# PlasmaControl/spectrogram-enhancement

Hardware: AMD Instinct MI355X
Metric: spectrograms/s (STFT+VAE-denoise fwd) at 1/2/4/8 GPUs; PSNR vs CPU ref (higher is better)
Workload: dtype fp16; 1 GPU; BASELINE config 5 per GPU: end-to-end STFT -> SVD -> autoencoder-denoise inference stream, 16,512-sample fp16 shots -> specgr 128x128 (256 hann / hop 128) -> denoiseSignal default -> 3-layer conv AE (16/32/64, 5x5) fp16 forward -> fp16 reconstructions (32,768 B per shot); shots_per_launch=2048, samples=16512, stft_dtype=fp32, svd_dtype=fp32 (fp64 small algebra), ae_dtype=fp16, parallelism=shot-sharded x1, streams_per_gpu=2

## Files before the change

### spectrogram-enhancement_amd/csrc/conv_rows.hip

```cpp
#include <hip/hip_runtime.h>

#include <algorithm>
#include <cstdint>
#include <mutex>
#include <string>
#include <type_traits>

#include "lds_dma.hpp"
#include "specenh.h"
#include "runtime.hpp"

namespace specenh {
int set_error(int code, const std::string& msg);

namespace {

typedef _Float16 f16x8 __attribute__((ext_vector_type(8)));
typedef __bf16 bf16x8 __attribute__((ext_vector_type(8)));
typedef float f32x4 __attribute__((ext_vector_type(4)));

template <typename T>
__device__ __forceinline__ f32x4 mfma(const uint4& a, const uint4& b, f32x4 acc) {
  if constexpr (__is_same(T, _Float16))
    return __builtin_amdgcn_mfma_f32_16x16x32_f16(__builtin_bit_cast(f16x8, a),
// ... 947 lines not shown
      f32x4 acc[4] = {bias, bias, bias, bias};
#pragma unroll
      for (int dy = DY0; dy <= DY1; ++dy) {
        const unsigned char* src = ring + ((g + dy - DY0) & 7) * C::ROWB;
#pragma unroll
        for (int dx = DY0; dx <= DY1; ++dx) {
          if (!C::any_tap(dy, dx)) continue;
          const uint4 b = *reinterpret_cast<const uint4*>(src + xo[dx - DY0]);
#pragma unroll
          for (int ph = 0; ph < 4; ++ph)
            if (C::tap(ph, dy, dx)) acc[ph] = mfma<T>(wf[C::tap_index(ph, dy, dx)], b, acc[ph]);
        }
      }
#pragma unroll
      for (int ph = 0; ph < 4; ++ph) pk[ph] = relu_pack4<T>(acc[ph]);
      const long long n = (long long)blockIdx.x + (long long)il * G;
      po = ((n * 2 * H + 2 * s) * OW + 2 * (16 * wx + m)) * CO + 16 * nb + 4 * kg;
      held = true;
    }
    if (mk[0] >= 0) wait_vmcnt_ss<15>(vmn - mk[0]);
    lds_barrier();
#pragma unroll
    for (int i = 0; i < LEAD; ++i) mk[i] = mk[i + 1];
    if (++s == SPI) { s = 0; ++il; }
    if (++sp == SPI) { sp = 0; ++ilp; }
  }
  store_held();
}

template <typename T, int CO, int W, int K>
hipError_t launch_convt_rows32(const CRArgs& a, hipStream_t st) {
  using C = TC32<CO, W, K>;
  constexpr int LEAD = 8 - C::NDY - 1 < 3 ? 8 - C::NDY - 1 : 3;
  const void* k = reinterpret_cast<const void*>(&convt_rows32_kernel<T, CO, W, K, LEAD>);
  static int per_cu[64] = {};
  int dev = 0;
  hipError_t e = hipGetDevice(&dev);
  if (e != hipSuccess) return e;
  if (dev < 0 || dev >= 64) dev = 0;
  if (per_cu[dev] == 0) {
    int pc = 0;
    e = hipOccupancyMaxActiveBlocksPerMultiprocessor(&pc, k, C::THREADS, C::LDS);
    if (e != hipSuccess) return e;
    per_cu[dev] = std::max(1, pc);
  }
  const long long grid = std::min<long long>(a.N, (long long)per_cu[dev] * device_cus());
  SPECENH_LAUNCH((convt_rows32_kernel<T, CO, W, K, LEAD>), dim3((unsigned)grid),
                 dim3(C::THREADS), C::LDS, st, a);
  return hipGetLastError();
}

constexpr int C1W = 128;
constexpr int C1CW = 72;
constexpr int C1ROW = 2 * C1CW;
constexpr int C1RING = 16;
constexpr int C1LDS = C1RING * C1ROW * 4;

template <typename T>
__global__ __launch_bounds__(256) void conv1_rows_pool_kernel(CRArgs a) {
  extern __shared__ __attribute__((aligned(16))) unsigned char ring_raw[];
  uint32_t* const ring = reinterpret_cast<uint32_t*>(ring_raw);
  const int tid = threadIdx.x, lane = tid & 63;
  const int wv = __builtin_amdgcn_readfirstlane(tid >> 6);
  const int m = lane & 15, kg = lane >> 4;
  const int H = a.H, SPI = H / 2 + 2, PPI = H + 4;
  const int G = gridDim.x;
  const int nimg = ((int)a.N - (int)blockIdx.x + G - 1) / G;
  const int S = nimg * SPI;

  for (int e = tid; e < C1RING * C1ROW; e += 256) ring[e] = 0u;
  uint4 w0, w1;
  {
    const T* __restrict__ Wg = reinterpret_cast<const T*>(a.w);
    uint32_t q0[4], q1[4];
#pragma unroll
    for (int i = 0; i < 4; ++i) {
      float v[4];
#pragma unroll
      for (int h = 0; h < 2; ++h) {
        const int kx = 2 * i + h;
        v[2 * h] = kx < 5 ? (float)Wg[(m * 5 + kg) * 5 + kx] : 0.f;
        v[2 * h + 1] = kx < 5 && kg == 0 ? (float)Wg[(m * 5 + 4) * 5 + kx] : 0.f;
      }
      q0[i] = pack2<T>(v[0], v[2]);
      q1[i] = pack2<T>(v[1], v[3]);
    }
    w0 = uint4{q0[0], q0[1], q0[2], q0[3]};
    w1 = uint4{q1[0], q1[1], q1[2], q1[3]};
  }
  const f32x4 bias = f32x4{a.b[4 * kg], a.b[4 * kg + 1], a.b[4 * kg + 2], a.b[4 * kg + 3]};

  const T* __restrict__ X = reinterpret_cast<const T*>(a.x);
  auto stage = [&](int pp) -> int {
    if (wv != 0) return 0;
    int nd = 0;
#pragma unroll
    for (int j = 0; j < 2; ++j) {
      const int pos = pp + j;
      const int il = pos / PPI, r = pos - il * PPI - 2;
      uint32_t* dst = ring + (pos & (C1RING - 1)) * C1ROW + 4;
      if (il < nimg && r >= 0 && r < H) {
        const long long n = (long long)blockIdx.x + (long long)il * G;
        if (lane < 16) lds_dma16(X + (n * H + r) * C1W + 8 * lane, dst);
        ++nd;
      } else if (lane < 16) {
        *reinterpret_cast<uint4*>(dst + 4 * lane) = uint4{0u, 0u, 0u, 0u};
      }
    }
    return nd;
  };
  auto shift = [&](int pp) {
    if (tid < 2 * C1CW) {
      const int j = tid / C1CW, i = tid - j * C1CW;
      uint32_t* row = ring + ((pp + j) & (C1RING - 1)) * C1ROW;
      const uint32_t lo = row[i], hi = row[i + 1];
      row[C1CW + i] = __builtin_amdgcn_alignbit(hi, lo, 16);
    }
  };
  __syncthreads();
  for (int pp = 0; pp < 10; pp += 2) stage(pp);
  asm volatile("s_waitcnt vmcnt(0)" ::: "memory");
  lds_barrier();
  shift(0); shift(2); shift(4);
  lds_barrier();

  const int wbase = 16 * wv + m + 3;
  auto bfrag = [&](int pos, int cb) -> uint4 {
    const uint32_t* row = ring + ((pos + kg) & (C1RING - 1)) * C1ROW + cb * C1CW + wbase;
    return uint4{row[0], row[1], row[2], row[3]};
  };
  T* __restrict__ O = reinterpret_cast<T*>(a.out);
  const int PW = C1W / 2, PH = H / 2;
  for (int g = 0; g < S; ++g) {
    const int nd = stage(2 * g + 10);
    shift(2 * g + 6);
    const int il = g / SPI, p = g - il * SPI;
    if (p < PH) {
      const int pb = 2 * g;
      f32x4 acc[2][2];
#pragma unroll
      for (int dy = 0; dy < 2; ++dy)
#pragma unroll
        for (int cb = 0; cb < 2; ++cb) {
          const uint4 b = bfrag(pb + dy, cb);
          uint4 b4 = bfrag(pb + dy + 4, cb);
          if (kg != 0) b4 = uint4{0u, 0u, 0u, 0u};
          acc[dy][cb] = mfma<T>(w0, b, bias);
          acc[dy][cb] = mfma<T>(w1, b4, acc[dy][cb]);
        }
      float v[4];
#pragma unroll
      for (int i = 0; i < 4; ++i)
        v[i] = fmaxf(fmaxf(fmaxf(acc[0][0][i], acc[0][1][i]), fmaxf(acc[1][0][i], acc[1][1][i])),
                     0.f);
      const long long n = (long long)blockIdx.x + (long long)il * G;
      *reinterpret_cast<uint2*>(O + ((n * PH + p) * PW + 16 * wv + m) * 16 + 4 * kg) =
          uint2{pack2<T>(v[0], v[1]), pack2<T>(v[2], v[3])};
    }
    if (wv == 0) {
      const int younger = nd + (p < PH ? 1 : 0);
      if (younger == 0) asm volatile("s_waitcnt vmcnt(0)" ::: "memory");
      else if (younger == 1) asm volatile("s_waitcnt vmcnt(1)" ::: "memory");
      else if (younger == 2) asm volatile("s_waitcnt vmcnt(2)" ::: "memory");
      else asm volatile("s_waitcnt vmcnt(3)" ::: "memory");
    }
    lds_barrier();
  }
}

template <typename T>
hipError_t launch_conv1_rows(const CRArgs& a, hipStream_t st) {
  const void* k = reinterpret_cast<const void*>(&conv1_rows_pool_kernel<T>);
  static int per_cu[64] = {};
  int dev = 0;
  hipError_t e = hipGetDevice(&dev);
  if (e != hipSuccess) return e;
  if (dev < 0 || dev >= 64) dev = 0;
  if (per_cu[dev] == 0) {
    int pc = 0;
    e = hipOccupancyMaxActiveBlocksPerMultiprocessor(&pc, k, 256, C1LDS);
    if (e != hipSuccess) return e;
    per_cu[dev] = std::max(1, pc);
  }
  const long long grid = std::min<long long>(a.N, (long long)per_cu[dev] * device_cus());
  SPECENH_LAUNCH(conv1_rows_pool_kernel<T>, dim3((unsigned)grid), dim3(256), C1LDS, st, a);
  return hipGetLastError();
}

struct E2Args {
  const void* x;
  const void* w1;
  const float* b1;
  const void* w2;
  const float* b2;
  void* out;
  int N, H;
};

constexpr int E2R1 = 32;
#ifndef SPECENH_ENC2_COPIES
#define SPECENH_ENC2_COPIES 4
#endif
constexpr int E2NC = SPECENH_ENC2_COPIES;
__host__ __device__ constexpr int E2CB(int c) {
  return E2NC == 4 ? (c == 0 ? 0 : c == 1 ? 72 : c == 2 ? 178 : 250) : c * C1CW;
}
constexpr int E2ROW = E2NC == 4 ? 352 : 2 * C1CW;
constexpr int E2RROWS = E2R1 + 2;
#ifndef SPECENH_ENC2_STAGGER
#define SPECENH_ENC2_STAGGER 0
#endif

template <typename T, int WPE>
__global__ __launch_bounds__(512) __attribute__((amdgpu_waves_per_eu(WPE)))
void enc2_rows_kernel(E2Args a) {
  using C = RC<16, 32, 64>;
  extern __shared__ __attribute__((aligned(16))) unsigned char lds[];
  unsigned char* const ring = lds;
  uint32_t* const ring1 = reinterpret_cast<uint32_t*>(lds + C::LDS);
  const int tid = threadIdx.x, lane = tid & 63;
  const int wv = __builtin_amdgcn_readfirstlane(tid >> 6);
  const int m = lane & 15, kg = lane >> 4;
  const int wx = wv % C::NWIN, nb = wv / C::NWIN;
  const int x0 = 16 * wx;
  const int H1 = a.H, H = H1 / 2;
  const int SPI = H / 2 + 1, PPI = H1 + 4;
  const int G = gridDim.x;
  const int nimg = ((int)a.N - (int)blockIdx.x + G - 1) / G;
  const int S = nimg * SPI + 1;

  for (int e = tid; e < (C::LDS + E2RROWS * E2ROW * 4) / 16; e += 512)
    reinterpret_cast<uint4*>(lds)[e] = uint4{0u, 0u, 0u, 0u};
  float* const btab = reinterpret_cast<float*>(lds + C::LDS + E2RROWS * E2ROW * 4);
  if (tid < 16) btab[tid] = a.b1[tid];
  else if (tid < 48) btab[tid] = a.b2[tid - 16];
  auto bias2_ld = [&]() { return *reinterpret_cast<const f32x4*>(btab + 16 + 16 * nb + 4 * kg); };

  uint4 wf[13];
  {
    const T* __restrict__ Wg = reinterpret_cast<const T*>(a.w2);
    const int co = 16 * nb + m, hi = kg >> 1, c8 = 8 * (kg & 1);
    auto tap = [&](int ky, int kx) {
      return *reinterpret_cast<const uint4*>(Wg + ((co * 5 + ky) * 5 + kx) * 16 + c8);
    };
#pragma unroll
    for (int ky = 0; ky < 5; ++ky) {
      wf[ky] = tap(ky, hi);
      wf[5 + ky] = tap(ky, 2 + hi);
    }
    wf[10] = tap(hi, 4);
    wf[11] = tap(2 + hi, 4);
    wf[12] = hi ? uint4{0u, 0u, 0u, 0u} : tap(4, 4);
  }

  const int boff = (x0 + m + (kg >> 1)) * 32 + 16 * (kg & 1);
  const int fo = (x0 + m + 4) * 32 + 16 * (kg & 1);
  const int foff = fo + (kg >> 1) * C::ROWB, foffw = fo - (kg >> 1) * 7 * C::ROWB;

  uint4 v0, v1;
  {
    const T* __restrict__ W1 = reinterpret_cast<const T*>(a.w1);
    uint32_t q0[4], q1[4];
#pragma unroll
    for (int i = 0; i < 4; ++i) {
      float v[4];
#pragma unroll
      for (int h = 0; h < 2; ++h) {
        const int kx = 2 * i + h;
        v[2 * h] = kx < 5 ? (float)W1[(m * 5 + kg) * 5 + kx] : 0.f;
        v[2 * h + 1] = kx < 5 && kg == 0 ? (float)W1[(m * 5 + 4) * 5 + kx] : 0.f;
      }
      q0[i] = pack2<T>(v[0], v[2]);
      q1[i] = pack2<T>(v[1], v[3]);
    }
    v0 = uint4{q0[0], q0[1], q0[2], q0[3]};
    v1 = uint4{q1[0], q1[1], q1[2], q1[3]};
  }
  resident_loads_landed();
  const int w1x = wv & 3, jr = wv >> 2;
  const int wbase = 16 * w1x + m + 3;
  const int p1 = 16 * w1x + m;
  const int c4hi = 2 * ((p1 + 3) & 1), w4 = p1 + 3 - ((p1 + 3) & 1);
  const int cbase0 = E2CB(c4hi) + w4, cbase1 = E2CB(1 + c4hi) + w4;

  const T* __restrict__ X = reinterpret_cast<const T*>(a.x);
  auto stage1_at = [&](int pos, int il, int y) -> int {
    uint32_t* dst = ring1 + (pos & (E2R1 - 1)) * E2ROW + 4;
    if (il < nimg && y >= 0 && y < H1) {
      const long long n = (long long)blockIdx.x + (long long)il * G;
      if (lane < 16) lds_dma16_s(X + (n * H1 + y) * C1W, 16u * lane, dst);
      return 1;
    }
    int z = 0;
    asm volatile("" : "+v"(z));
    if (lane < 16) *reinterpret_cast<uint4*>(dst + 4 * lane) = uint4{(uint32_t)z, (uint32_t)z, (uint32_t)z, (uint32_t)z};
    return 0;
  };
  auto stage1 = [&](int pp) -> int {
    if (wv >= 4) return 0;
    const int pos = pp + wv;
    const int il = pos / PPI;
    return stage1_at(pos, il, pos - il * PPI - 2);
  };
  auto shift1 = [&](int pp) {
    constexpr int NW = E2NC == 4 ? C1CW - 2 : C1CW;
    if (tid < 4 * NW) {
      const int j = tid / NW, i = tid - j * NW;
      uint32_t* row = ring1 + ((pp + j) & (E2R1 - 1)) * E2ROW;
      const uint32_t r0 = row[i], r1 = row[i + 1];
      row[E2CB(1) + i] = __builtin_amdgcn_alignbit(r1, r0, 16);
      if constexpr (E2NC == 4) {
        const uint32_t r2 = row[i + 2];
        row[E2CB(2) + i] = r1;
        row[E2CB(3) + i] = __builtin_amdgcn_alignbit(r2, r1, 16);
      }
    }
  };
  auto run_at = [&](const uint32_t* row, int cb) -> uint4 {
    if constexpr (E2NC == 4) {
      typedef __attribute__((address_space(3))) const volatile unsigned long long lds_u64;
      const lds_u64* r = (const lds_u64*)(row + (cb ? cbase1 : cbase0));
      const unsigned long long lo = r[0], hi = r[1];
      return uint4{(uint32_t)lo, (uint32_t)(lo >> 32), (uint32_t)hi, (uint32_t)(hi >> 32)};
    } else {
      const uint32_t* r = row + cb * C1CW + wbase;
      return uint4{r[0], r[1], r[2], r[3]};
    }
  };
  auto bfrag = [&](int pos, int cb) -> uint4 {
    return run_at(ring1 + ((pos + kg) & (E2R1 - 1)) * E2ROW, cb);
  };
  auto bfrag4 = [&](int pos, int cb) -> uint4 {
    const uint32_t* zrow = ring1 + (E2NC == 4 ? E2R1 + 1 - (pos & 1) : E2R1) * E2ROW;
    return run_at(kg == 0 ? ring1 + (pos & (E2R1 - 1)) * E2ROW : zrow, cb);
  };
  auto produce = [&](int g2, int il, int q2) {
    const int r = 2 * q2 + jr;
    const int pb = 4 * g2 + 2 * jr;
    float v[4] = {0.f, 0.f, 0.f, 0.f};
    const f32x4 bias1 = *reinterpret_cast<const f32x4*>(btab + 4 * kg);
#pragma unroll
    for (int dy = 0; dy < 2; ++dy)
#pragma unroll
      for (int cb = 0; cb < 2; ++cb) {
        const uint4 b = bfrag(pb + dy, cb);
        const uint4 b4 = bfrag4(pb + dy + 4, cb);
        f32x4 acc1 = mfma<T>(v0, b, bias1);
        acc1 = mfma<T>(v1, b4, acc1);
#pragma unroll
        for (int i = 0; i < 4; ++i) v[i] = fmaxf(v[i], acc1[i]);
      }
    const bool real = il < nimg && r < H;
    const uint2 pk = real ? uint2{pack2<T>(v[0], v[1]), pack2<T>(v[2], v[3])} : uint2{0u, 0u};
    *reinterpret_cast<uint2*>(ring + ((2 * g2 + jr) & 7) * C::ROWB + (16 * w1x + m + 2) * 32 +
                              8 * kg) = pk;
  };

  __syncthreads();
  for (int pp = 0; pp < 32; pp += 4) stage1(pp);
  asm volatile("s_waitcnt vmcnt(0)" ::: "memory");
  lds_barrier();
  for (int pp = 0; pp < 16; pp += 4) shift1(pp);
  lds_barrier();
  produce(0, 0, 0);
  produce(1, 1 / SPI, 1 % SPI);
  lds_barrier();

  f32x4 acc[6];
#pragma unroll
  for (int i = 0; i < 6; ++i) acc[i] = bias2_ld();
  T* __restrict__ O = reinterpret_cast<T*>(a.out);
  const int PW = 32, PHh = H / 2;
  int c_1 = 0, c_2 = 0;
  auto fdiv = [](int x, int d) { return x >= 0 ? x / d : -((-x + d - 1) / d); };
  int ilA = fdiv(-2, SPI), qA = -2 - ilA * SPI;
  int qC = 0;
  int ilB = 2 / SPI, qB = 2 - ilB * SPI;
  int ilD = (32 + wv) / PPI, rD = 32 + wv - ilD * PPI;
  auto adv = [](int& il, int& q, int by, int per) {
    q += by;
    if (q >= per) { q -= per; ++il; }
  };

  auto step = [&](auto ic, const int s) {
    constexpr int I = decltype(ic)::value;
    auto slot = [](int d) { return (2 * I + d + 12) % 6; };
    int ns = 0;
    {
      f32x4& r0 = acc[slot(-4)];
      f32x4& r1 = acc[slot(-3)];
      {
        const int il = ilA, q = qA;
        if (il >= 0 && il < nimg && q < PHh) {
          ns = 1;
          float v[4];
#pragma unroll
          for (int i = 0; i < 4; ++i) v[i] = fmaxf(max_pair(fmaxf(r0[i], r1[i])), 0.f);
          const long long n = (long long)blockIdx.x + (long long)il * G;
          const long long o = ((n * PHh + q) * PW + (x0 + m) / 2) * 32 + 16 * nb + 4 * kg;
          *reinterpret_cast<uint2*>(O + o) = uint2{pack2<T>(v[0], v[1]), pack2<T>(v[2], v[3])};
        }
      }
      const f32x4 bias = bias2_ld();
      r0 = bias;
// ... 20 lines not shown
      for (int ky = 0; ky < 5; ++ky) {
        f32x4& ac = acc[slot(j + 2 - ky)];
        ac = mfma<T>(wf[5 + ky], b2, ac);
      }
      acc[slot(j + 2)] = mfma<T>(wf[10], bF, acc[slot(j + 2)]);
      acc[slot(j)] = mfma<T>(wf[11], bF, acc[slot(j)]);
      acc[slot(j - 2)] = mfma<T>(wf[12], bF, acc[slot(j - 2)]);
      if (j == 0) {
        uint4 bT = *reinterpret_cast<const uint4*>(ring + ((2 * s) & 7) * C::ROWB + fo);
        if (kg < 2 || q != 0) bT = uint4{0u, 0u, 0u, 0u};
        acc[slot(1)] = mfma<T>(wf[10], bT, acc[slot(1)]);
      }
    }
    };
    if (SPECENH_ENC2_STAGGER && wv >= 4) {
      conv2_rows();
      produce(s + 2, ilB, qB);
    } else {
      produce(s + 2, ilB, qB);
      conv2_rows();
    }
    if (wv < 4) {
      const int younger = c_2 + c_1 + ns + nd;
      if (younger >= 6) {
        asm volatile("s_waitcnt vmcnt(6)" ::: "memory");
      } else switch (younger) {
        case 0: asm volatile("s_waitcnt vmcnt(0)" ::: "memory"); break;
        case 1: asm volatile("s_waitcnt vmcnt(1)" ::: "memory"); break;
        case 2: asm volatile("s_waitcnt vmcnt(2)" ::: "memory"); break;
        case 3: asm volatile("s_waitcnt vmcnt(3)" ::: "memory"); break;
        case 4: asm volatile("s_waitcnt vmcnt(4)" ::: "memory"); break;
        case 5: asm volatile("s_waitcnt vmcnt(5)" ::: "memory"); break;
        default: asm volatile("s_waitcnt vmcnt(6)" ::: "memory"); break;
      }
    }
    c_2 = c_1;
    c_1 = ns + nd;
    adv(ilA, qA, 1, SPI);
    qC = qC + 1 == SPI ? 0 : qC + 1;
    adv(ilB, qB, 1, SPI);
    adv(ilD, rD, 4, PPI);
    lds_barrier();
  };
  int s = 0;
  for (; s + 3 <= S; s += 3) {
    step(std::integral_constant<int, 0>{}, s);
    step(std::integral_constant<int, 1>{}, s + 1);
    step(std::integral_constant<int, 2>{}, s + 2);
  }
  if (s < S) step(std::integral_constant<int, 0>{}, s);
  if (s + 1 < S) step(std::integral_constant<int, 1>{}, s + 1);
}

constexpr int E2LDS = RC<16, 32, 64>::LDS + E2RROWS * E2ROW * 4 + 48 * 4;

template <typename T, int WPE>
hipError_t launch_enc2_wpe(const E2Args& a, hipStream_t st) {
  const void* k = reinterpret_cast<const void*>(&enc2_rows_kernel<T, WPE>);
  static int per_cu[64] = {};
  int dev = 0;
  hipError_t e = hipGetDevice(&dev);
  if (e != hipSuccess) return e;
  if (dev < 0 || dev >= 64) dev = 0;
  if (per_cu[dev] == 0) {
    int pc = 0;
    e = hipOccupancyMaxActiveBlocksPerMultiprocessor(&pc, k, 512, E2LDS);
    if (e != hipSuccess) return e;
    per_cu[dev] = std::max(1, pc);
  }
  const long long grid = std::min<long long>(a.N, (long long)per_cu[dev] * device_cus());
  SPECENH_LAUNCH((enc2_rows_kernel<T, WPE>), dim3((unsigned)grid), dim3(512), E2LDS, st, a);
  return hipGetLastError();
}

template <typename T>
hipError_t launch_enc2(const E2Args& a, hipStream_t st) {
  return variant(V_ENC2_WPE2) ? launch_enc2_wpe<T, 2>(a, st) : launch_enc2_wpe<T, 4>(a, st);
}

}

int conv_rows_pool(int dtype, const void* x, int N, int H, int W, int CI, const void* w,
                   const float* b, int CO, int K, void* out, hipStream_t st, bool* launched) {
  *launched = false;
  if (variant(V_CONV_NO_ROWS) != 0 || N <= 0 || H < 2 || (H & 1) || !b) return SPECENH_OK;
  if ((long long)N * H * W * CI >= (1ll << 31)) return SPECENH_OK;
  CRArgs a{};
  a.x = x; a.w = w; a.b = b; a.out = out; a.N = N; a.H = H;
  hipError_t e = hipSuccess;
  const bool f16 = dtype == SPECENH_DTYPE_F16;
  if (dtype != SPECENH_DTYPE_F16 && dtype != SPECENH_DTYPE_BF16) return SPECENH_OK;
  if (CI == 16 && CO == 32 && W == 64 && K == 5)
    e = f16 ? launch_rows<_Float16, 16, 32, 64>(a, st) : launch_rows<__bf16, 16, 32, 64>(a, st);
  else if (CI == 32 && CO == 64 && W == 32 && K == 5)
    e = f16 ? launch_rows<_Float16, 32, 64, 32>(a, st) : launch_rows<__bf16, 32, 64, 32>(a, st);
  else if (CI == 32 && CO == 32 && W == 64 && K == 5)
    e = f16 ? launch_rows<_Float16, 32, 32, 64>(a, st) : launch_rows<__bf16, 32, 32, 64>(a, st);
  else if (CI == 32 && CO == 32 && W == 64 && K == 3)
    e = f16 ? launch_rows<_Float16, 32, 32, 64, 3>(a, st) : launch_rows<__bf16, 32, 32, 64, 3>(a, st);
  else
    return SPECENH_OK;
  if (e != hipSuccess) return set_error(SPECENH_EHIP, std::string("conv_rows: ") + hipGetErrorString(e));
  *launched = true;
  return SPECENH_OK;
}

}

namespace specenh {

int convt_rows(int dtype, const void* x, int N, int H, int W, int CI, const void* w,
               const float* b, int CO, int K, void* out, hipStream_t st, bool* launched) {
  *launched = false;
  if (variant(V_CONVT_NO_ROWS) != 0 || N <= 0 || H <= 0 || !b) return SPECENH_OK;
  if (dtype != SPECENH_DTYPE_F16 && dtype != SPECENH_DTYPE_BF16) return SPECENH_OK;
  if ((long long)N * 4 * H * W * CO >= (1ll << 31)) return SPECENH_OK;
  CRArgs a{};
  a.x = x; a.w = w; a.b = b; a.out = out; a.N = N; a.H = H;
  const bool f16 = dtype == SPECENH_DTYPE_F16;
  hipError_t e;
  if (CI == 32) {
    if (CO != 32 || W != 32) return SPECENH_OK;
    if (K == 3) e = f16 ? launch_convt_rows32<_Float16, 32, 32, 3>(a, st) : launch_convt_rows32<__bf16, 32, 32, 3>(a, st);
    else if (K == 5) e = f16 ? launch_convt_rows32<_Float16, 32, 32, 5>(a, st) : launch_convt_rows32<__bf16, 32, 32, 5>(a, st);
    else if (K == 7) e = f16 ? launch_convt_rows32<_Float16, 32, 32, 7>(a, st) : launch_convt_rows32<__bf16, 32, 32, 7>(a, st);
    else return SPECENH_OK;
    if (e != hipSuccess) return set_error(SPECENH_EHIP, std::string("convt_rows32: ") + hipGetErrorString(e));
    *launched = true;
    return SPECENH_OK;
  }
// ... 5 lines not shown
  else if (CO == 64 && W == 16)
    e = f16 ? launch_convt_rows<_Float16, 64, 16>(a, st) : launch_convt_rows<__bf16, 64, 16>(a, st);
  else if (CO == 32 && W == 32)
    e = f16 ? launch_convt_rows<_Float16, 32, 32>(a, st) : launch_convt_rows<__bf16, 32, 32>(a, st);
  else
    return SPECENH_OK;
  if (e != hipSuccess) return set_error(SPECENH_EHIP, std::string("convt_rows: ") + hipGetErrorString(e));
  *launched = true;
  return SPECENH_OK;
}

}

namespace specenh {

int conv1_rows_pool(int dtype, const void* x, int N, int H, int W, const void* w,
                    const float* b, int CO, void* out, hipStream_t st, bool* launched) {
  *launched = false;
  if (variant(V_CONV1_NO_ROWS) != 0 || N <= 0 || H < 2 || (H & 1) || W != C1W || CO != 16 || !b)
    return SPECENH_OK;
  if (dtype != SPECENH_DTYPE_F16 && dtype != SPECENH_DTYPE_BF16) return SPECENH_OK;
  if (((uintptr_t)x & 15) || (long long)N * H * W >= (1ll << 31)) return SPECENH_OK;
  CRArgs a{};
  a.x = x; a.w = w; a.b = b; a.out = out; a.N = N; a.H = H;
  const hipError_t e = dtype == SPECENH_DTYPE_F16 ? launch_conv1_rows<_Float16>(a, st)
                                                  : launch_conv1_rows<__bf16>(a, st);
  if (e != hipSuccess) return set_error(SPECENH_EHIP, std::string("conv1_rows: ") + hipGetErrorString(e));
  *launched = true;
  return SPECENH_OK;
}

}

extern "C" int specenh_encoder2(int dtype, const void* x, int N, int H, int W, const void* w1_gemm,
                                const float* b1, int CO1, const void* w2_gemm, const float* b2,
                                int CO2, int k, void* out, void* stream) {
  using namespace specenh;
  if (N < 0 || H <= 0 || W <= 0) return set_error(SPECENH_EINVAL, "bad input shape");
  if (dtype != SPECENH_DTYPE_F16 && dtype != SPECENH_DTYPE_BF16)
    return set_error(SPECENH_EUNSUPPORTED, "fused encoder: fp16 / bf16 only");
  if (W != C1W || CO1 != 16 || CO2 != 32 || k != 5 || (H & 3))
    return set_error(SPECENH_EUNSUPPORTED,
                     "fused encoder: Conv2D(16, 5) + pool + Conv2D(32, 5) + pool on 128-wide "
                     "one-channel images, height a multiple of 4");
  if (N == 0) return SPECENH_OK;
  if (!x || !w1_gemm || !b1 || !w2_gemm || !b2 || !out) return set_error(SPECENH_EINVAL, "null pointer");
  if (((uintptr_t)x & 15) || (long long)N * H * W >= (1ll << 31))
    return set_error(SPECENH_EINVAL, "input must be 16-byte aligned and below 2^31 elements");
  E2Args a{};
  a.x = x; a.w1 = w1_gemm; a.b1 = b1; a.w2 = w2_gemm; a.b2 = b2; a.out = out; a.N = N; a.H = H;
  hipStream_t st = (hipStream_t)stream;
  static std::once_flag once;
  std::call_once(once, [] {
    const void* const ks[4] = {reinterpret_cast<const void*>(&enc2_rows_kernel<_Float16, 4>),
                               reinterpret_cast<const void*>(&enc2_rows_kernel<__bf16, 4>),
                               reinterpret_cast<const void*>(&enc2_rows_kernel<_Float16, 2>),
                               reinterpret_cast<const void*>(&enc2_rows_kernel<__bf16, 2>)};
    for (const void* k : ks)
      (void)hipFuncSetAttribute(k, hipFuncAttributeMaxDynamicSharedMemorySize, E2LDS);
  });
  const hipError_t e = dtype == SPECENH_DTYPE_F16 ? launch_enc2<_Float16>(a, st)
                                                  : launch_enc2<__bf16>(a, st);
  if (e != hipSuccess) return set_error(SPECENH_EHIP, std::string("encoder2: ") + hipGetErrorString(e));
  return SPECENH_OK;
}
```

### spectrogram-enhancement_amd/csrc/runtime.hip

```cpp
#include "runtime.hpp"

#include <atomic>
#include <cstdlib>
#include <cstring>
#include <mutex>
#include <string>

#include "specenh.h"

namespace specenh {
int set_error(int code, const std::string& msg);

namespace {

struct VariantName {
  const char* name;
  int dflt;
};
constexpr VariantName kVariants[V_COUNT] = {
    {"CONVT_PAIR", 0},      {"PATCH_NO_WL", 0},      {"PATCH_NO_K5", 0},
    {"PATCH_WSPLIT", -1},   {"CONV_NO_S2", 0},       {"CONV_NO_PATCH", 0},
    {"CONV_NO_C1MFMA", 0},  {"CONV_NO_NARROW", 0},   {"WGRAD_GENERIC", 0},
    {"WGRAD_NO_CO1", 0},    {"WGRAD_PERPHASE", 0},   {"SVD_GRAM_TILES", 0},
    {"TAIL_TILES", 0},      {"DECODER_UNFUSED", 0},  {"SVD_NO_TOP1", 0},
    {"CONV_NO_ROWS", 0},    {"CONVT_NO_ROWS", 0},    {"CONV1_NO_ROWS", 0},
    {"ENCODER_UNFUSED", 0},  {"STFT_NO_HOLD", 0},    {"D3_MAP", 0},
    {"ENC2_WPE2", 0},        {"CONVT_SHARED_RING", 0}, {"SVD_RECON_VALU", 0},
    {"ROWS_SHORT_LEAD", 0},  {"SVD_GRAM_F32", 0},
    {"SVD_RECON_BLOCKS", 0}, {"CONVT_PG", 0}, {"SVD_GZ_ROWS", 0}, {"EIG_SPLIT", 0}, {"CO1_VALU", 0},
    {"C1_MASK_MFMA", 1}, {"S2_MIN_NT", 2}, {"PATCH_MIN_WG", 512}, {"WGRAD_WG", 1024}, {"WGRAD_C1_TILES", 4},
    {"EIG_GRID", 32}, {"ROWS_BANDS", -1},
};

std::atomic<int> g_variant[V_COUNT];
std::once_flag g_variant_once;

void init_variants() {
  for (int i = 0; i < V_COUNT; ++i) {
    int v = kVariants[i].dflt;
    std::string env = std::string("SPECENH_") + kVariants[i].name;
    if (const char* s = std::getenv(env.c_str()); s && *s) v = std::atoi(s);
    g_variant[i].store(v, std::memory_order_relaxed);
  }
}

int variant_index(const char* name) {
  if (!name) return -1;
  if (std::strncmp(name, "SPECENH_", 8) == 0) name += 8;
  for (int i = 0; i < V_COUNT; ++i)
    if (std::strcmp(name, kVariants[i].name) == 0) return i;
  return -1;
}

constexpr int kMaxDevices = 64;
std::atomic<int> g_cus[kMaxDevices];

constexpr int kRing = 256;
thread_local const void* g_ring[kRing];
thread_local long long g_launches = 0;

}

int variant(Variant v) {
  std::call_once(g_variant_once, init_variants);
  return g_variant[v].load(std::memory_order_relaxed);
}

int device_cus() {
  int dev = 0;
  if (hipGetDevice(&dev) != hipSuccess || dev < 0 || dev >= kMaxDevices) return 256;
  int c = g_cus[dev].load(std::memory_order_relaxed);
  if (c > 0) return c;
  if (hipDeviceGetAttribute(&c, hipDeviceAttributeMultiprocessorCount, dev) != hipSuccess || c <= 0)
    c = 256;
  g_cus[dev].store(c, std::memory_order_relaxed);
  return c;
}

void note_launch(const void* kernel) { g_ring[g_launches++ % kRing] = kernel; }

}

extern "C" {

// ... 67 lines not shown
```

### spectrogram-enhancement_amd/csrc/runtime.hpp

```cpp
#pragma once

#include <hip/hip_runtime.h>

namespace specenh {

enum Variant : int {
  V_CONVT_PAIR = 0,
  V_PATCH_NO_WL,
  V_PATCH_NO_K5,
  V_PATCH_WSPLIT,
  V_CONV_NO_S2,
  V_CONV_NO_PATCH,
  V_CONV_NO_C1MFMA,
  V_CONV_NO_NARROW,
  V_WGRAD_GENERIC,
  V_WGRAD_NO_CO1,
  V_WGRAD_PERPHASE,
  V_SVD_GRAM_TILES,
  V_TAIL_TILES,
  V_DECODER_UNFUSED,
  V_SVD_NO_TOP1,
  V_CONV_NO_ROWS,
  V_CONVT_NO_ROWS,
  V_CONV1_NO_ROWS,
  V_ENCODER_UNFUSED,
  V_STFT_NO_HOLD,
  V_D3_MAP,
  V_ENC2_WPE2,
  V_CONVT_SHARED_RING,
  V_SVD_RECON_VALU,
  V_ROWS_SHORT_LEAD,
  V_SVD_GRAM_F32,
  V_SVD_RECON_BLOCKS,
  V_CONVT_PG,
  V_SVD_GZ_ROWS,
  V_EIG_SPLIT,
  V_CO1_VALU,
  V_C1_MASK_MFMA,
  V_S2_MIN_NT,
  V_PATCH_MIN_WG,
  V_WGRAD_WG,
  V_WGRAD_C1_TILES,
  V_EIG_GRID,
  V_ROWS_BANDS,
  V_COUNT
};

int variant(Variant v);

int device_cus();

void note_launch(const void* kernel);

}

#define SPECENH_LAUNCH(K, ...)                                        \
  do {                                                                \
    ::specenh::note_launch(reinterpret_cast<const void*>(&K));        \
    hipLaunchKernelGGL(K, __VA_ARGS__);                               \
  } while (0)
```

### spectrogram-enhancement_amd/csrc/svd_denoise.hip

```cpp
#include <hip/hip_runtime.h>

#include <algorithm>
#include <cmath>
#include <cstdlib>
#include <string>
#include <vector>

#include "fft_common.hpp"
#include "specenh.h"
#include "runtime.hpp"

namespace specenh {
int set_error(int code, const std::string& msg);

typedef float f32x16 __attribute__((ext_vector_type(16)));

struct XView {
  const float* base;
  long long batch_stride;
  long long sk, si;
};

__global__ __launch_bounds__(256) void gram_kernel(XView x, int K, int r, float* G,
                                                   int ntiles_side) {
// ... 2764 lines not shown
  if (e != hipSuccess) return e;
  SPECENH_LAUNCH((recon_kernel<KP, TO>), dim3((Kr + RB - 1) / RB, (unsigned)nb), dim3(256),
                     lds, st, xb, Kr, r, V, K, lo, hi, comp, only, reinterpret_cast<TO*>(out),
                     ob, osk, osi);
  return hipGetLastError();
}

template <typename TO>
hipError_t launch_recon_k(int KP, XView xb, int Kr, int r, const float* V, int K, int lo,
                          int hi, int comp, const int* only, void* out, long long ob,
                          long long osk, long long osi, long long nb, hipStream_t st) {
  switch (KP) {
#define SPECENH_RC(n)                                                                          \
  case n:                                                                                      \
    return launch_recon_t<n, TO>(xb, Kr, r, V, K, lo, hi, comp, only, out, ob, osk, osi, nb, \
                                 st);
    SPECENH_RC(8) SPECENH_RC(16) SPECENH_RC(24) SPECENH_RC(32) SPECENH_RC(40) SPECENH_RC(48)
#undef SPECENH_RC
    default: return hipErrorInvalidValue;
  }
}

hipError_t launch_recon(int KP, XView xb, int Kr, int r, const float* V, int K, int lo, int hi,
                        int comp, const int* only, void* out, long long ob, long long osk,
                        long long osi, long long nb, hipStream_t st, int odt = SPECENH_DTYPE_F32) {
  if (odt == SPECENH_DTYPE_F16)
    return launch_recon_k<_Float16>(KP, xb, Kr, r, V, K, lo, hi, comp, only, out, ob, osk, osi, nb, st);
  if (odt == SPECENH_DTYPE_BF16)
    return launch_recon_k<__bf16>(KP, xb, Kr, r, V, K, lo, hi, comp, only, out, ob, osk, osi, nb, st);
  return launch_recon_k<float>(KP, xb, Kr, r, V, K, lo, hi, comp, only, out, ob, osk, osi, nb, st);
}

size_t dtype_size(int dt) { return dt == SPECENH_DTYPE_F32 ? 4 : 2; }

struct EigLayout {
  int r;
  long long ld;
  size_t per_matrix() const {
    return (size_t)r * r * 8 + 3 * (size_t)r * 8 + 4 * (size_t)r * ld * 8 + 4 * 4 + 8;
  }
  static constexpr size_t kCapBytes = 1ull << 30;
  long long chunk(long long batch) const {
    const long long c = (long long)(kCapBytes / per_matrix());
    return std::max(1LL, std::min(batch, c));
  }
  size_t bytes(long long batch) const { return (size_t)chunk(batch) * per_matrix() + 256; }
};
EigLayout eig_layout(int r) { return EigLayout{r, (long long)(r / 2 + 2)}; }

#ifndef SPECENH_EIG_MERGED
#define SPECENH_EIG_MERGED 1
#endif
template <typename TO>
__global__ __launch_bounds__(256) void eig_fallback_kernel(
    XView x, int Kr, int r, double* G, int nts, double* dg, double* eg, double* taug, int lo,
    int hi, double* Z, double* fac, long long ld, int* kinfo, TO* out, long long out_bstride,
    long long osk, long long osi, const int* only, long long nmat) {
  const int ntri = nts * (nts + 1) / 2, nkb = (Kr + RB - 1) / RB;
  for (long long b = blockIdx.x; b < nmat; b += gridDim.x) {
    if (!only[b]) continue;
    for (int t = 0; t < ntri; ++t) {
      gram64_one(x, Kr, r, G, nts, b, t);
      __syncthreads();
    }
    __threadfence();
    __syncthreads();
    tridiag_one(G, r, dg, eg, taug, b);
    __threadfence();
    __syncthreads();
    eigvec_one(G, dg, eg, taug, r, lo, hi, nullptr, Z, fac, ld, kinfo, b);
    __threadfence();
    __syncthreads();
    for (int kb = 0; kb < nkb; ++kb) {
      recon_eig_one<TO>(x, Kr, r, Z, ld, kinfo, out, out_bstride, osk, osi, b, kb);
      __syncthreads();
    }
  }
}

template <typename TO>
hipError_t launch_recon_eig_t(XView xb, int Kr, int r, const double* Z, long long ld,
                              const int* kinfo, void* out, long long ob, long long osk,
                              long long osi, long long nb, hipStream_t st, const int* only) {
  const size_t lds = (size_t)RB * (r + 1) * 4 + (size_t)r * 33 * 4 + (size_t)RB * 33 * 4;
  hipError_t e = hipFuncSetAttribute((const void*)recon_eig_kernel<TO>,
                                     hipFuncAttributeMaxDynamicSharedMemorySize, (int)lds);
  if (e != hipSuccess) return e;
  const unsigned gm = only ? (unsigned)std::min<long long>(nb, 2LL * device_cus()) : (unsigned)nb;
  SPECENH_LAUNCH(recon_eig_kernel<TO>, dim3((Kr + RB - 1) / RB, gm), dim3(256), lds, st, xb, Kr,
                 r, Z, ld, kinfo, reinterpret_cast<TO*>(out), ob, osk, osi, only, nb);
  return hipGetLastError();
}

hipError_t launch_recon_eig(int odt, XView xb, int Kr, int r, const double* Z, long long ld,
                            const int* kinfo, void* out, long long ob, long long osk,
                            long long osi, long long nb, hipStream_t st, const int* only) {
  if (odt == SPECENH_DTYPE_F16)
    return launch_recon_eig_t<_Float16>(xb, Kr, r, Z, ld, kinfo, out, ob, osk, osi, nb, st, only);
  if (odt == SPECENH_DTYPE_BF16)
    return launch_recon_eig_t<__bf16>(xb, Kr, r, Z, ld, kinfo, out, ob, osk, osi, nb, st, only);
  return launch_recon_eig_t<float>(xb, Kr, r, Z, ld, kinfo, out, ob, osk, osi, nb, st, only);
}

template <typename TO>
hipError_t launch_eig_fallback_t(XView xb, int Kr, int r, double* G, int nts, double* dg,
                                 double* eg, double* taug, int lo, int hi, double* Z,
                                 double* fac, long long ld, int* kinfo, void* out, long long ob,
                                 long long osk, long long osi, const int* only, long long nb,
                                 unsigned gm, hipStream_t st) {
  const size_t lds = (size_t)RB * (r + 1) * 4 + (size_t)r * 33 * 4 + (size_t)RB * 33 * 4;
  hipError_t e = hipFuncSetAttribute((const void*)eig_fallback_kernel<TO>,
                                     hipFuncAttributeMaxDynamicSharedMemorySize, (int)lds);
  if (e != hipSuccess) return e;
  SPECENH_LAUNCH(eig_fallback_kernel<TO>, dim3(gm), dim3(256), lds, st, xb, Kr, r, G, nts, dg,
                 eg, taug, lo, hi, Z, fac, ld, kinfo, reinterpret_cast<TO*>(out), ob, osk, osi,
                 only, nb);
  return hipGetLastError();
}

hipError_t launch_eig_fallback(int odt, XView xb, int Kr, int r, double* G, int nts, double* dg,
                               double* eg, double* taug, int lo, int hi, double* Z, double* fac,
                               long long ld, int* kinfo, void* out, long long ob, long long osk,
                               long long osi, const int* only, long long nb, unsigned gm,
                               hipStream_t st) {
  if (odt == SPECENH_DTYPE_F16)
    return launch_eig_fallback_t<_Float16>(xb, Kr, r, G, nts, dg, eg, taug, lo, hi, Z, fac, ld,
                                           kinfo, out, ob, osk, osi, only, nb, gm, st);
  if (odt == SPECENH_DTYPE_BF16)
// ... 348 lines not shown
```

Measured before the change: 1.969 million spectrograms/s.

## Replace conv1 pixel-shift LDS copies with shifted-weight MFMA fragments

The conv1 and fused enc2 kernels now, by default, encode the odd-pixel shift in the weight fragments (kslot_up realigns the k-slots) instead of building shifted copies of each input row in LDS. This drops the shift/copy passes and shrinks the LDS ring rows, at the cost of four weight fragments per lane. In enc2 with WPE=4 the fragments live in an LDS table to save registers. Separately, the eig fallback kernel now scans the 'only' flags 256 at a time with a ballot and processes only flagged matrices instead of testing each index serially. The old path stays selectable through a CONV1_PIXSHIFT variant.

```diff
diff --git a/spectrogram-enhancement_amd/csrc/conv_rows.hip b/spectrogram-enhancement_amd/csrc/conv_rows.hip
--- a/spectrogram-enhancement_amd/csrc/conv_rows.hip
+++ b/spectrogram-enhancement_amd/csrc/conv_rows.hip
@@ -1023,12 +1023,60 @@
 
 constexpr int C1W = 128;
 constexpr int C1CW = 72;
-constexpr int C1ROW = 2 * C1CW;
 constexpr int C1RING = 16;
-constexpr int C1LDS = C1RING * C1ROW * 4;
+template <bool PIX>
+struct C1L {
+  static constexpr int ROW = PIX ? 2 * C1CW : 80;
+  static constexpr int LDS = C1RING * ROW * 4;
+};
 
 template <typename T>
+__device__ __forceinline__ void conv1_weights(const T* __restrict__ Wg, int m, int kg,
+                                              uint4 (&w)[4]) {
+  const int ky[4] = {kg, kg == 0 ? 4 : -1, kg - 1, kg == 0 ? 3 : kg == 1 ? 4 : -1};
+#pragma unroll
+  for (int f = 0; f < 4; ++f) {
+    uint32_t q[4];
+#pragma unroll
+    for (int i = 0; i < 4; ++i) {
+      float v[2];
+#pragma unroll
+      for (int h = 0; h < 2; ++h) {
+        const int kx = 2 * i + h;
+        v[h] = kx < 5 && ky[f] >= 0 ? (float)Wg[(m * 5 + ky[f]) * 5 + kx] : 0.f;
+      }
+      q[i] = pack2<T>(v[0], v[1]);
+    }
+    w[f] = uint4{q[0], q[1], q[2], q[3]};
+  }
+}
+
+__device__ __forceinline__ uint4 kslot_up(const uint4& w) {
+  return uint4{w.x << 16, __builtin_amdgcn_alignbit(w.y, w.x, 16),
+               __builtin_amdgcn_alignbit(w.z, w.y, 16), __builtin_amdgcn_alignbit(w.w, w.z, 16)};
+}
+
+template <typename T>
+__device__ __forceinline__ void conv1_pool4(const uint4 (&w)[4], const uint4& Ba,
+                                            const uint4& Bb, const f32x4& bias, float (&v)[4]) {
+#pragma unroll
+  for (int i = 0; i < 4; ++i) v[i] = 0.f;
+#pragma unroll
+  for (int dy = 0; dy < 2; ++dy)
+#pragma unroll
+    for (int cb = 0; cb < 2; ++cb) {
+      const uint4 wa = cb ? kslot_up(w[2 * dy]) : w[2 * dy];
+      const uint4 wb = cb ? kslot_up(w[2 * dy + 1]) : w[2 * dy + 1];
+      f32x4 acc = mfma<T>(wa, Ba, bias);
+      acc = mfma<T>(wb, Bb, acc);
+#pragma unroll
+      for (int i = 0; i < 4; ++i) v[i] = fmaxf(v[i], acc[i]);
+    }
+}
+
+template <typename T, bool PIX>
 __global__ __launch_bounds__(256) void conv1_rows_pool_kernel(CRArgs a) {
+  constexpr int C1ROW = C1L<PIX>::ROW;
   extern __shared__ __attribute__((aligned(16))) unsigned char ring_raw[];
   uint32_t* const ring = reinterpret_cast<uint32_t*>(ring_raw);
   const int tid = threadIdx.x, lane = tid & 63;
@@ -1040,8 +1088,10 @@
   const int S = nimg * SPI;
 
   for (int e = tid; e < C1RING * C1ROW; e += 256) ring[e] = 0u;
-  uint4 w0, w1;
-  {
+  uint4 w0{}, w1{}, ws[4]{};
+  if constexpr (!PIX) {
+    conv1_weights<T>(reinterpret_cast<const T*>(a.w), m, kg, ws);
+  } else {
     const T* __restrict__ Wg = reinterpret_cast<const T*>(a.w);
     uint32_t q0[4], q1[4];
 #pragma unroll
@@ -1081,6 +1131,7 @@
     return nd;
   };
   auto shift = [&](int pp) {
+    if constexpr (!PIX) return;
     if (tid < 2 * C1CW) {
       const int j = tid / C1CW, i = tid - j * C1CW;
       uint32_t* row = ring + ((pp + j) & (C1RING - 1)) * C1ROW;
@@ -1108,22 +1159,29 @@
     const int il = g / SPI, p = g - il * SPI;
     if (p < PH) {
       const int pb = 2 * g;
-      f32x4 acc[2][2];
-#pragma unroll
-      for (int dy = 0; dy < 2; ++dy)
-#pragma unroll
-        for (int cb = 0; cb < 2; ++cb) {
-          const uint4 b = bfrag(pb + dy, cb);
-          uint4 b4 = bfrag(pb + dy + 4, cb);
-          if (kg != 0) b4 = uint4{0u, 0u, 0u, 0u};
-          acc[dy][cb] = mfma<T>(w0, b, bias);
-          acc[dy][cb] = mfma<T>(w1, b4, acc[dy][cb]);
-        }
       float v[4];
-#pragma unroll
-      for (int i = 0; i < 4; ++i)
-        v[i] = fmaxf(fmaxf(fmaxf(acc[0][0][i], acc[0][1][i]), fmaxf(acc[1][0][i], acc[1][1][i])),
-                     0.f);
+      if constexpr (!PIX) {
+        const uint4 ba = bfrag(pb, 0);
+        uint4 bb = bfrag(pb + 4, 0);
+        if (kg >= 2) bb = uint4{0u, 0u, 0u, 0u};
+        conv1_pool4<T>(ws, ba, bb, bias, v);
+      } else {
+        f32x4 acc[2][2];
+#pragma unroll
+        for (int dy = 0; dy < 2; ++dy)
+#pragma unroll
+          for (int cb = 0; cb < 2; ++cb) {
+            const uint4 b = bfrag(pb + dy, cb);
+            uint4 b4 = bfrag(pb + dy + 4, cb);
+            if (kg != 0) b4 = uint4{0u, 0u, 0u, 0u};
+            acc[dy][cb] = mfma<T>(w0, b, bias);
+            acc[dy][cb] = mfma<T>(w1, b4, acc[dy][cb]);
+          }
+#pragma unroll
+        for (int i = 0; i < 4; ++i)
+          v[i] = fmaxf(fmaxf(fmaxf(acc[0][0][i], acc[0][1][i]), fmaxf(acc[1][0][i], acc[1][1][i])),
+                       0.f);
+      }
       const long long n = (long long)blockIdx.x + (long long)il * G;
       *reinterpret_cast<uint2*>(O + ((n * PH + p) * PW + 16 * wv + m) * 16 + 4 * kg) =
           uint2{pack2<T>(v[0], v[1]), pack2<T>(v[2], v[3])};
@@ -1139,9 +1197,10 @@
   }
 }
 
-template <typename T>
-hipError_t launch_conv1_rows(const CRArgs& a, hipStream_t st) {
-  const void* k = reinterpret_cast<const void*>(&conv1_rows_pool_kernel<T>);
+template <typename T, bool PIX>
+hipError_t launch_conv1_rows_v(const CRArgs& a, hipStream_t st) {
+  constexpr int C1LDS = C1L<PIX>::LDS;
+  const void* k = reinterpret_cast<const void*>(&conv1_rows_pool_kernel<T, PIX>);
   static int per_cu[64] = {};
   int dev = 0;
   hipError_t e = hipGetDevice(&dev);
@@ -1154,8 +1213,14 @@
     per_cu[dev] = std::max(1, pc);
   }
   const long long grid = std::min<long long>(a.N, (long long)per_cu[dev] * device_cus());
-  SPECENH_LAUNCH(conv1_rows_pool_kernel<T>, dim3((unsigned)grid), dim3(256), C1LDS, st, a);
+  SPECENH_LAUNCH((conv1_rows_pool_kernel<T, PIX>), dim3((unsigned)grid), dim3(256), C1LDS, st, a);
   return hipGetLastError();
+}
+
+template <typename T>
+hipError_t launch_conv1_rows(const CRArgs& a, hipStream_t st) {
+  return variant(V_CONV1_PIXSHIFT) ? launch_conv1_rows_v<T, true>(a, st)
+                                   : launch_conv1_rows_v<T, false>(a, st);
 }
 
 struct E2Args {
@@ -1169,23 +1234,25 @@
 };
 
 constexpr int E2R1 = 32;
-#ifndef SPECENH_ENC2_COPIES
-#define SPECENH_ENC2_COPIES 4
-#endif
-constexpr int E2NC = SPECENH_ENC2_COPIES;
-__host__ __device__ constexpr int E2CB(int c) {
-  return E2NC == 4 ? (c == 0 ? 0 : c == 1 ? 72 : c == 2 ? 178 : 250) : c * C1CW;
-}
-constexpr int E2ROW = E2NC == 4 ? 352 : 2 * C1CW;
-constexpr int E2RROWS = E2R1 + 2;
+template <bool PIX>
+struct E2L {
+  static constexpr int CB(int c) { return c == 0 ? 0 : c == 1 ? 72 : c == 2 ? 178 : 250; }
+  static constexpr int ROW = PIX ? 352 : C1L<false>::ROW;
+  static constexpr int RROWS = PIX ? E2R1 + 2 : E2R1 + 1;
+  static constexpr int WTAB = PIX ? 0 : 4 * 64 * 16;
+  static constexpr int BTAB = RC<16, 32, 64>::LDS + RROWS * ROW * 4;
+  static constexpr int LDS = BTAB + 48 * 4 + WTAB;
+};
 #ifndef SPECENH_ENC2_STAGGER
 #define SPECENH_ENC2_STAGGER 0
 #endif
 
-template <typename T, int WPE>
+template <typename T, int WPE, bool PIX>
 __global__ __launch_bounds__(512) __attribute__((amdgpu_waves_per_eu(WPE)))
 void enc2_rows_kernel(E2Args a) {
   using C = RC<16, 32, 64>;
+  using L = E2L<PIX>;
+  constexpr int E2ROW = L::ROW;
   extern __shared__ __attribute__((aligned(16))) unsigned char lds[];
   unsigned char* const ring = lds;
   uint32_t* const ring1 = reinterpret_cast<uint32_t*>(lds + C::LDS);
@@ -1200,9 +1267,9 @@
   const int nimg = ((int)a.N - (int)blockIdx.x + G - 1) / G;
   const int S = nimg * SPI + 1;
 
-  for (int e = tid; e < (C::LDS + E2RROWS * E2ROW * 4) / 16; e += 512)
+  for (int e = tid; e < L::BTAB / 16; e += 512)
     reinterpret_cast<uint4*>(lds)[e] = uint4{0u, 0u, 0u, 0u};
-  float* const btab = reinterpret_cast<float*>(lds + C::LDS + E2RROWS * E2ROW * 4);
+  float* const btab = reinterpret_cast<float*>(lds + L::BTAB);
   if (tid < 16) btab[tid] = a.b1[tid];
   else if (tid < 48) btab[tid] = a.b2[tid - 16];
   auto bias2_ld = [&]() { return *reinterpret_cast<const f32x4*>(btab + 16 + 16 * nb + 4 * kg); };
@@ -1228,8 +1295,17 @@
   const int fo = (x0 + m + 4) * 32 + 16 * (kg & 1);
   const int foff = fo + (kg >> 1) * C::ROWB, foffw = fo - (kg >> 1) * 7 * C::ROWB;
 
-  uint4 v0, v1;
-  {
+  constexpr bool W1LDS = WPE == 4;
+  constexpr int NRES = W1LDS ? 0 : 4;
+  uint4 v0{}, v1{}, w1f[4]{};
+  uint4* const wtab = reinterpret_cast<uint4*>(lds + L::BTAB + 48 * 4);
+  if constexpr (!PIX) {
+    conv1_weights<T>(reinterpret_cast<const T*>(a.w1), m, kg, w1f);
+    if constexpr (W1LDS) {
+#pragma unroll
+      for (int f = 0; f < 4; ++f) wtab[f * 64 + lane] = w1f[f];
+    }
+  } else {
     const T* __restrict__ W1 = reinterpret_cast<const T*>(a.w1);
     uint32_t q0[4], q1[4];
 #pragma unroll
@@ -1252,19 +1328,22 @@
   const int wbase = 16 * w1x + m + 3;
   const int p1 = 16 * w1x + m;
   const int c4hi = 2 * ((p1 + 3) & 1), w4 = p1 + 3 - ((p1 + 3) & 1);
-  const int cbase0 = E2CB(c4hi) + w4, cbase1 = E2CB(1 + c4hi) + w4;
+  const int cbase0 = L::CB(c4hi) + w4, cbase1 = L::CB(1 + c4hi) + w4;
 
   const T* __restrict__ X = reinterpret_cast<const T*>(a.x);
   auto stage1_at = [&](int pos, int il, int y) -> int {
     uint32_t* dst = ring1 + (pos & (E2R1 - 1)) * E2ROW + 4;
+    int z = 0;
+    asm volatile("" : "+v"(z));
+    const int ln = PIX ? lane
+                       : (int)__builtin_amdgcn_mbcnt_hi(
+                             ~0u, __builtin_amdgcn_mbcnt_lo(~0u, (uint32_t)z));
     if (il < nimg && y >= 0 && y < H1) {
       const long long n = (long long)blockIdx.x + (long long)il * G;
-      if (lane < 16) lds_dma16_s(X + (n * H1 + y) * C1W, 16u * lane, dst);
+      if (ln < 16) lds_dma16_s(X + (n * H1 + y) * C1W, 16u * ln, dst);
       return 1;
     }
-    int z = 0;
-    asm volatile("" : "+v"(z));
-    if (lane < 16) *reinterpret_cast<uint4*>(dst + 4 * lane) = uint4{(uint32_t)z, (uint32_t)z, (uint32_t)z, (uint32_t)z};
+    if (ln < 16) *reinterpret_cast<uint4*>(dst + 4 * ln) = uint4{(uint32_t)z, (uint32_t)z, (uint32_t)z, (uint32_t)z};
     return 0;
   };
   auto stage1 = [&](int pp) -> int {
@@ -1274,27 +1353,25 @@
     return stage1_at(pos, il, pos - il * PPI - 2);
   };
   auto shift1 = [&](int pp) {
-    constexpr int NW = E2NC == 4 ? C1CW - 2 : C1CW;
+    if constexpr (!PIX) return;
+    constexpr int NW = C1CW - 2;
     if (tid < 4 * NW) {
       const int j = tid / NW, i = tid - j * NW;
       uint32_t* row = ring1 + ((pp + j) & (E2R1 - 1)) * E2ROW;
-      const uint32_t r0 = row[i], r1 = row[i + 1];
-      row[E2CB(1) + i] = __builtin_amdgcn_alignbit(r1, r0, 16);
-      if constexpr (E2NC == 4) {
-        const uint32_t r2 = row[i + 2];
-        row[E2CB(2) + i] = r1;
-        row[E2CB(3) + i] = __builtin_amdgcn_alignbit(r2, r1, 16);
-      }
+      const uint32_t r0 = row[i], r1 = row[i + 1], r2 = row[i + 2];
+      row[L::CB(1) + i] = __builtin_amdgcn_alignbit(r1, r0, 16);
+      row[L::CB(2) + i] = r1;
+      row[L::CB(3) + i] = __builtin_amdgcn_alignbit(r2, r1, 16);
     }
   };
   auto run_at = [&](const uint32_t* row, int cb) -> uint4 {
-    if constexpr (E2NC == 4) {
+    if constexpr (PIX) {
       typedef __attribute__((address_space(3))) const volatile unsigned long long lds_u64;
       const lds_u64* r = (const lds_u64*)(row + (cb ? cbase1 : cbase0));
       const unsigned long long lo = r[0], hi = r[1];
       return uint4{(uint32_t)lo, (uint32_t)(lo >> 32), (uint32_t)hi, (uint32_t)(hi >> 32)};
     } else {
-      const uint32_t* r = row + cb * C1CW + wbase;
+      const uint32_t* r = row + wbase;
       return uint4{r[0], r[1], r[2], r[3]};
     }
   };
@@ -1302,25 +1379,41 @@
     return run_at(ring1 + ((pos + kg) & (E2R1 - 1)) * E2ROW, cb);
   };
   auto bfrag4 = [&](int pos, int cb) -> uint4 {
-    const uint32_t* zrow = ring1 + (E2NC == 4 ? E2R1 + 1 - (pos & 1) : E2R1) * E2ROW;
+    const uint32_t* zrow = ring1 + (E2R1 + 1 - (pos & 1)) * E2ROW;
     return run_at(kg == 0 ? ring1 + (pos & (E2R1 - 1)) * E2ROW : zrow, cb);
+  };
+  auto bfragb = [&](int pos) -> uint4 {
+    return run_at(ring1 + (kg < 2 ? (pos + kg) & (E2R1 - 1) : E2R1) * E2ROW, 0);
   };
   auto produce = [&](int g2, int il, int q2) {
     const int r = 2 * q2 + jr;
     const int pb = 4 * g2 + 2 * jr;
     float v[4] = {0.f, 0.f, 0.f, 0.f};
     const f32x4 bias1 = *reinterpret_cast<const f32x4*>(btab + 4 * kg);
-#pragma unroll
-    for (int dy = 0; dy < 2; ++dy)
-#pragma unroll
-      for (int cb = 0; cb < 2; ++cb) {
-        const uint4 b = bfrag(pb + dy, cb);
-        const uint4 b4 = bfrag4(pb + dy + 4, cb);
-        f32x4 acc1 = mfma<T>(v0, b, bias1);
-        acc1 = mfma<T>(v1, b4, acc1);
-#pragma unroll
-        for (int i = 0; i < 4; ++i) v[i] = fmaxf(v[i], acc1[i]);
-      }
+    if constexpr (!PIX) {
+#pragma unroll
+      for (int f = 0; f < 4; ++f) {
+        if (f < NRES)
+          asm volatile("" : "+v"(w1f[f].x), "+v"(w1f[f].y), "+v"(w1f[f].z), "+v"(w1f[f].w));
+        else
+          w1f[f] = wtab[f * 64 + lane];
+      }
+      const uint4 ba = bfrag(pb, 0);
+      const uint4 bb = bfragb(pb + 4);
+      conv1_pool4<T>(w1f, ba, bb, bias1, v);
+    } else {
+#pragma unroll
+      for (int dy = 0; dy < 2; ++dy)
+#pragma unroll
+        for (int cb = 0; cb < 2; ++cb) {
+          const uint4 b = bfrag(pb + dy, cb);
+          const uint4 b4 = bfrag4(pb + dy + 4, cb);
+          f32x4 acc1 = mfma<T>(v0, b, bias1);
+          acc1 = mfma<T>(v1, b4, acc1);
+#pragma unroll
+          for (int i = 0; i < 4; ++i) v[i] = fmaxf(v[i], acc1[i]);
+        }
+    }
     const bool real = il < nimg && r < H;
     const uint2 pk = real ? uint2{pack2<T>(v[0], v[1]), pack2<T>(v[2], v[3])} : uint2{0u, 0u};
     *reinterpret_cast<uint2*>(ring + ((2 * g2 + jr) & 7) * C::ROWB + (16 * w1x + m + 2) * 32 +
@@ -1447,11 +1540,10 @@
   if (s + 1 < S) step(std::integral_constant<int, 1>{}, s + 1);
 }
 
-constexpr int E2LDS = RC<16, 32, 64>::LDS + E2RROWS * E2ROW * 4 + 48 * 4;
-
-template <typename T, int WPE>
+template <typename T, int WPE, bool PIX>
 hipError_t launch_enc2_wpe(const E2Args& a, hipStream_t st) {
-  const void* k = reinterpret_cast<const void*>(&enc2_rows_kernel<T, WPE>);
+  constexpr int E2LDS = E2L<PIX>::LDS;
+  const void* k = reinterpret_cast<const void*>(&enc2_rows_kernel<T, WPE, PIX>);
   static int per_cu[64] = {};
   int dev = 0;
   hipError_t e = hipGetDevice(&dev);
@@ -1464,13 +1556,17 @@
     per_cu[dev] = std::max(1, pc);
   }
   const long long grid = std::min<long long>(a.N, (long long)per_cu[dev] * device_cus());
-  SPECENH_LAUNCH((enc2_rows_kernel<T, WPE>), dim3((unsigned)grid), dim3(512), E2LDS, st, a);
+  SPECENH_LAUNCH((enc2_rows_kernel<T, WPE, PIX>), dim3((unsigned)grid), dim3(512), E2LDS, st, a);
   return hipGetLastError();
 }
 
 template <typename T>
 hipError_t launch_enc2(const E2Args& a, hipStream_t st) {
-  return variant(V_ENC2_WPE2) ? launch_enc2_wpe<T, 2>(a, st) : launch_enc2_wpe<T, 4>(a, st);
+  if (variant(V_CONV1_PIXSHIFT))
+    return variant(V_ENC2_WPE2) ? launch_enc2_wpe<T, 2, true>(a, st)
+                                : launch_enc2_wpe<T, 4, true>(a, st);
+  return variant(V_ENC2_WPE2) ? launch_enc2_wpe<T, 2, false>(a, st)
+                              : launch_enc2_wpe<T, 4, false>(a, st);
 }
 
 }
@@ -1582,12 +1678,18 @@
   hipStream_t st = (hipStream_t)stream;
   static std::once_flag once;
   std::call_once(once, [] {
-    const void* const ks[4] = {reinterpret_cast<const void*>(&enc2_rows_kernel<_Float16, 4>),
-                               reinterpret_cast<const void*>(&enc2_rows_kernel<__bf16, 4>),
-                               reinterpret_cast<const void*>(&enc2_rows_kernel<_Float16, 2>),
-                               reinterpret_cast<const void*>(&enc2_rows_kernel<__bf16, 2>)};
-    for (const void* k : ks)
-      (void)hipFuncSetAttribute(k, hipFuncAttributeMaxDynamicSharedMemorySize, E2LDS);
+    auto set = [](auto pix) {
+      constexpr bool PIX = decltype(pix)::value;
+      const void* const ks[4] = {
+          reinterpret_cast<const void*>(&enc2_rows_kernel<_Float16, 4, PIX>),
+          reinterpret_cast<const void*>(&enc2_rows_kernel<__bf16, 4, PIX>),
+          reinterpret_cast<const void*>(&enc2_rows_kernel<_Float16, 2, PIX>),
+          reinterpret_cast<const void*>(&enc2_rows_kernel<__bf16, 2, PIX>)};
+      for (const void* k : ks)
+        (void)hipFuncSetAttribute(k, hipFuncAttributeMaxDynamicSharedMemorySize, E2L<PIX>::LDS);
+    };
+    set(std::false_type{});
+    set(std::true_type{});
   });
   const hipError_t e = dtype == SPECENH_DTYPE_F16 ? launch_enc2<_Float16>(a, st)
                                                   : launch_enc2<__bf16>(a, st);
diff --git a/spectrogram-enhancement_amd/csrc/runtime.hip b/spectrogram-enhancement_amd/csrc/runtime.hip
--- a/spectrogram-enhancement_amd/csrc/runtime.hip
+++ b/spectrogram-enhancement_amd/csrc/runtime.hip
@@ -29,7 +29,7 @@
     {"ROWS_SHORT_LEAD", 0},  {"SVD_GRAM_F32", 0},
     {"SVD_RECON_BLOCKS", 0}, {"CONVT_PG", 0}, {"SVD_GZ_ROWS", 0}, {"EIG_SPLIT", 0}, {"CO1_VALU", 0},
     {"C1_MASK_MFMA", 1}, {"S2_MIN_NT", 2}, {"PATCH_MIN_WG", 512}, {"WGRAD_WG", 1024}, {"WGRAD_C1_TILES", 4},
-    {"EIG_GRID", 32}, {"ROWS_BANDS", -1},
+    {"EIG_GRID", 32}, {"ROWS_BANDS", -1}, {"CONV1_PIXSHIFT", 0},
 };
 
 std::atomic<int> g_variant[V_COUNT];
diff --git a/spectrogram-enhancement_amd/csrc/runtime.hpp b/spectrogram-enhancement_amd/csrc/runtime.hpp
--- a/spectrogram-enhancement_amd/csrc/runtime.hpp
+++ b/spectrogram-enhancement_amd/csrc/runtime.hpp
@@ -43,6 +43,7 @@
   V_WGRAD_C1_TILES,
   V_EIG_GRID,
   V_ROWS_BANDS,
+  V_CONV1_PIXSHIFT,
   V_COUNT
 };
 
diff --git a/spectrogram-enhancement_amd/csrc/svd_denoise.hip b/spectrogram-enhancement_amd/csrc/svd_denoise.hip
--- a/spectrogram-enhancement_amd/csrc/svd_denoise.hip
+++ b/spectrogram-enhancement_amd/csrc/svd_denoise.hip
@@ -2840,28 +2840,57 @@
 #define SPECENH_EIG_MERGED 1
 #endif
 template <typename TO>
+__device__ __forceinline__ void eig_fallback_one(
+    XView x, int Kr, int r, double* G, int nts, double* dg, double* eg, double* taug, int lo,
+    int hi, double* Z, double* fac, long long ld, int* kinfo, TO* out, long long out_bstride,
+    long long osk, long long osi, long long b, int ntri, int nkb) {
+  for (int t = 0; t < ntri; ++t) {
+    gram64_one(x, Kr, r, G, nts, b, t);
+    __syncthreads();
+  }
+  __threadfence();
+  __syncthreads();
+  tridiag_one(G, r, dg, eg, taug, b);
+  __threadfence();
+  __syncthreads();
+  eigvec_one(G, dg, eg, taug, r, lo, hi, nullptr, Z, fac, ld, kinfo, b);
+  __threadfence();
+  __syncthreads();
+  for (int kb = 0; kb < nkb; ++kb) {
+    recon_eig_one<TO>(x, Kr, r, Z, ld, kinfo, out, out_bstride, osk, osi, b, kb);
+    __syncthreads();
+  }
+}
+
+template <typename TO>
 __global__ __launch_bounds__(256) void eig_fallback_kernel(
     XView x, int Kr, int r, double* G, int nts, double* dg, double* eg, double* taug, int lo,
     int hi, double* Z, double* fac, long long ld, int* kinfo, TO* out, long long out_bstride,
     long long osk, long long osi, const int* only, long long nmat) {
   const int ntri = nts * (nts + 1) / 2, nkb = (Kr + RB - 1) / RB;
-  for (long long b = blockIdx.x; b < nmat; b += gridDim.x) {
-    if (!only[b]) continue;
-    for (int t = 0; t < ntri; ++t) {
-      gram64_one(x, Kr, r, G, nts, b, t);
-      __syncthreads();
-    }
-    __threadfence();
+  __shared__ unsigned long long s_flagged[2][4];
+  int par = 0;
+  for (long long i0 = 0; blockIdx.x + i0 * gridDim.x < nmat; i0 += 256, par ^= 1) {
+    const long long bt = blockIdx.x + (i0 + threadIdx.x) * gridDim.x;
+    const int mine = bt < nmat ? only[bt] : 0;
+    const unsigned long long bal = __ballot(mine != 0);
+    if ((threadIdx.x & 63) == 0) s_flagged[par][threadIdx.x >> 6] = bal;
     __syncthreads();
-    tridiag_one(G, r, dg, eg, taug, b);
-    __threadfence();
-    __syncthreads();
-    eigvec_one(G, dg, eg, taug, r, lo, hi, nullptr, Z, fac, ld, kinfo, b);
-    __threadfence();
-    __syncthreads();
-    for (int kb = 0; kb < nkb; ++kb) {
-      recon_eig_one<TO>(x, Kr, r, Z, ld, kinfo, out, out_bstride, osk, osi, b, kb);
-      __syncthreads();
+    unsigned long long masks[4];
+    for (int w = 0; w < 4; ++w) {
+      const unsigned long long m = s_flagged[par][w];
+      masks[w] = ((unsigned long long)__builtin_amdgcn_readfirstlane((unsigned)(m >> 32)) << 32) |
+                 (unsigned)__builtin_amdgcn_readfirstlane((unsigned)m);
+    }
+    for (int w = 0; w < 4; ++w) {
+      unsigned long long mask = masks[w];
+      while (mask) {
+        const int bit = __ffsll((long long)mask) - 1;
+        mask &= mask - 1;
+        eig_fallback_one<TO>(x, Kr, r, G, nts, dg, eg, taug, lo, hi, Z, fac, ld, kinfo, out,
+                             out_bstride, osk, osi, blockIdx.x + (i0 + w * 64 + bit) * gridDim.x,
+                             ntri, nkb);
+      }
     }
   }
 }
```

Result: no change. 1.989 million spectrograms/s (median of 6 runs) (+1.0%).
